# XiSHEN0220/RANSAC-Flow

Hardware: AMD Instinct MI355X
Metric: aligned image-pairs/sec @480×640, 1/2/4/8 MI355X; max-abs flow Δ vs ref (higher is better)
Workload: dtype f32

## Files before the change

include/rfx_api.h:

```cpp
#ifndef RFX_API_H
#define RFX_API_H

#include <stddef.h>
#include <stdint.h>

#ifdef __cplusplus
extern "C" {
#endif

#define RFX_OK 0
#define RFX_E_ARG (-1)
#define RFX_E_LIMIT (-2)

#define RFX_ACT_NONE 0
#define RFX_ACT_RELU 1
#define RFX_ACT_SIGMOID 2

const char* rfx_version(void);

#define RFX_ABI_VERSION 14
int rfx_abi_version(void);

int rfx_group_begin(void);
int rfx_group_end(void* stream);
int rfx_group_abort(void);
int rfx_group_side_streams(int enable);

int rfx_conv2d_f32(const float* in, const float* wT, const int32_t* ktab, const float* scale,
                   const float* shift, const float* residual, float* out, int N, int Cin, int Hin,
                   int Win, int Cout, int KH, int KW, int stride, int pad, int act, void* stream);

int rfx_conv2d_tile_variant(int N, int Cout, int Hout, int Wout);

int rfx_conv2d_kernel_id(int N, int Cin, int Cout, int KH, int KW, int stride, int pad, int Hout, int Wout);

int rfx_conv3x3_f32(const float* in, const float* wP, const float* scale, const float* shift, const float* residual,
                    float* out, int N, int Cin, int H, int W, int Cout, int act, int k_chunk, void* stream);
int rfx_conv3x3_kernel_id(int N, int Cin, int Cout, int H, int W, int k_chunk);
int rfx_conv3x3_s2_f32(const float* in, const float* wP, const float* scale, const float* shift, const float* residual,
                       float* out, int N, int Cin, int H, int W, int Cout, int act, void* stream);

int rfx_conv3x3_conv1x1_kernel_id(int N, int H, int W, int Cmid);
int rfx_conv3x3_conv1x1_f32(const float* in, const float* wP2, const float* scale2, const float* shift2, int act2,
                            const float* wQ3, const float* scale3, const float* shift3, const float* residual, int act3,
                            float* out, int N, int Cin, int H, int W, int Cmid, int Cexp, void* stream);

int rfx_maxpool2d_f32(const float* in, float* out, int NC, int Hin, int Win, int k, int stride,
                      int pad, void* stream);

int rfx_blurpool2d_f32(const float* in, float* out, int NC, int Hin, int Win, int stride, void* stream);

int rfx_maxblurpool2d_f32(const float* in, float* out, int NC, int Hin, int Win, int stride, void* stream);

int rfx_stem_conv3x3_maxblur_f32(const float* in, const float* wT, const float* scale, const float* shift, float* out,
                                 int N, int H, int W, int Cout, void* stream);

int rfx_stem_conv7x7_maxpool_f32(const float* in, const float* wT, const float* scale, const float* shift, float* out,
                                 int N, int H, int W, int Cout, void* stream);

int rfx_l2norm_nchw_f32(const float* in, float* out, int N, int C, int HW, long long out_batch_stride,
                        long long out_chan_stride, void* stream);
int rfx_l2norm_nchw_scatter_f32(const float* in, float* out, int N, int C, int HW, const long long* dst_off,
                                long long out_chan_stride, void* stream);

int rfx_flow_head_f32(const float* logits, float* flow, int N, int K, int rows, int cols, void* stream);

int rfx_resize_bilinear_f32(const float* in, float* out, int NC, int Hin, int Win, int Hout, int Wout,
                            int align_corners, void* stream);

int rfx_lanczos_pass_u8(const uint8_t* in, uint8_t* out, int N, int inH, int inW, int outH, int outW, int C,
                        const int32_t* bounds, const int32_t* weights, int ksize, int vertical, int row_offset,
                        void* stream);

int rfx_u8_to_f32_chw(const uint8_t* in, float* raw, float* norm, int N, int H, int W, const float* mean3_host,
                      const float* std3_host, void* stream);

int rfx_copy_cols_f32(const float* src, float* dst, long long rows, int w_src, int w_dst, void* stream);

int rfx_corr_neigh_f32(const float* x, const float* y, float* out, int N, int C, int H, int W, int K,
                       void* stream);
int rfx_corr_neigh_variant_f32(const float* x, const float* y, float* out, int N, int C, int H, int W, int K,
                               int variant, void* stream);

int rfx_corr_neigh_bidir_f32(const float* x, const float* y, float* out_xy, float* out_yx, int N, int C, int H, int W, int K,
                             void* stream);
int rfx_corr_timing(int enable);
int rfx_corr_timing_collect(float* us_out, int cap);

int rfx_warp_grid_f32(const float* Hm, float* grid, int B, int h, int w, void* stream);

int rfx_grid_sample_f32(const float* in, const float* grid, float* out, int N, int C, int Hi, int Wi,
                        int Ho, int Wo, int align_corners, void* stream);

int rfx_compose_flow_f32(const float* flowDown, const float* coarseGrid, float* flow12, float* inb,
                         float* flowUp, int N, int hd, int wd, int Hc, int Wc, int H, int W, int clamp, void* stream);

int rfx_flow_grad_clamp_f32(const float* flowCoarse, const float* grid, float* flowGrad, float* flow, int B, int H, int W,
                            int grid_batch, void* stream);

int rfx_merge_multi_h_f32(const float* flow, const float* match12, long long match12_stride, const float* cyc,
                          const float* inb, int n, long long HW, float th, int multiH, float* flowGlobal,
                          float* matchGlobal, uint8_t* binary, void* stream);

int rfx_match_score_f32(const float* match12, long long match12_stride, const float* cyc, const float* inb, int n,
                        long long HW, float* score, void* stream);

size_t rfx_remove_small_cc_ws_bytes(int N, int H, int W);
int rfx_remove_small_cc_f32(const float* in, float* out, int N, int H, int W, float match_th, int max_area, void* ws,
                            void* stream);

size_t rfx_remove_small_cc_ragged_ws_bytes(long long total_px);
int rfx_remove_small_cc_ragged_f32(const float* in, float* out, const long long* match_off, const int32_t* dims, int n_active,
                                   long long total_px, long long max_hw, float match_th, void* ws, void* stream);

size_t rfx_mutual_nn_ws_bytes(int nA, int nB);
int rfx_mutual_nn_f32(const float* featA, int ldA, int nA, const float* featB, int ldB, int nB, int C,
                      const float* maskB, int64_t* idx1, int64_t* idx2, int32_t* count, void* ws, int score_chunk,
                      void* stream);

int rfx_mutual_nn_batched_f32(const float* featA, int ldA, int nA, long long strideA, const float* featB, int ldB,
                              int nB, long long strideB, int C, const float* maskB, int64_t* idx1, int64_t* idx2,
                              int32_t* count, void* ws, int batch, int score_chunk, void* stream);

int rfx_mutual_nn_ragged_f32(const float* featA, int ldA, const float* featB, int ldB, const int32_t* nA, const int32_t* nB,
                             int maxNA, int maxNB, int C, const float* maskB, int64_t* idx1, int64_t* idx2, int cap,
                             int32_t* count, void* ws, int batch, int score_chunk, void* stream);

int rfx_dlt4_homography(const float* X, const float* Y, int N, float* Hout, void* stream);

int rfx_prediction_f32(const float* match1, const float* match2, int n, const float* Hs, int N, float* err,
                       void* stream);

int rfx_score_hypotheses(const float* match1, const float* match2, int n, const int64_t* samples, int N,
                         float tol, float* Hout, int64_t* counts, uint8_t* flags_out, void* ws, void* stream);

size_t rfx_ransac_ws_bytes(int n, int N);
int rfx_ransac_h4(const float* match1, const float* match2, int n, const int64_t* samples, int N,
                  float tol, float* bestH, uint8_t* inlier, int32_t* result, void* ws, void* stream);

size_t rfx_ransac_batched_ws_bytes(int cap, int N, int batch);
int rfx_ransac_h4_batched(const float* match1, const float* match2, const int32_t* n, int cap, const int64_t* samples,
                          int N, float tol, float* bestH, uint8_t* inlier, int32_t* result, void* ws, int batch,
                          void* stream);

int rfx_ransac_h4_batched_stage(const float* match1, const float* match2, const int32_t* n, int cap, const int64_t* samples,
                                int N, float tol, float* bestH, uint8_t* inlier, int32_t* result, void* ws, int batch,
                                int stages, void* stream);
int rfx_ransac_degenerate_list(const void* ws, int cap, int N, int batch, int32_t* idx, int32_t* count, int kcap, void* stream);
int rfx_ransac_patch_h(void* ws, int cap, int N, int batch, const int32_t* idx, const int32_t* count, const float* Hpatch,
                       int kcap, void* stream);
int rfx_ransac_degenerate_gather(const void* ws, const float* match1, const float* match2, const int32_t* n, int cap,
                                 const int64_t* samples, int N, int batch, int32_t* idx, int32_t* count, int32_t* off,
                                 int32_t* off_host, float* xy_rows, int row_cap, void* stream);
int rfx_ransac_patch_h_rows(void* ws, int cap, int N, int batch, const int32_t* idx, const int32_t* count, const int32_t* off,
                            const float* H_rows, int row_cap, void* stream);
int rfx_dlt4_homography_flags(const float* X, const float* Y, int N, float* Hout, uint8_t* flags, void* stream);

int rfx_gather_matches_f32(const int64_t* idx1, const int64_t* idx2, const int32_t* n, int cap, const float* xa,
                           const float* ya, const float* xb, const float* yb, float* match1, float* match2, int batch,
                           void* stream);

int rfx_gather_matches_ragged_f32(const int64_t* idx1, const int64_t* idx2, const int32_t* n, int cap, const float* xa,
                                  const float* ya, const long long* offA, const float* xb, const float* yb, const long long* offB,
                                  float* match1, float* match2, int batch, void* stream);

int rfx_draw_samples_i64(const int32_t* n, int64_t* samples, int N, int batch, uint64_t seed, uint64_t stream_id,
                         const int32_t* pair_ids, void* stream);

int rfx_keep_mask_f32(const float* mask, const float* bg, const int32_t* active, int n_active, int h, int w, int rt, int ct,
                      float* keep, void* stream);

int rfx_filter_matches_f32(const int64_t* idx1, const int64_t* idx2, const int32_t* count, int cap, const int32_t* active,
                           int n_active, const float* mask, const float* bg, int h, int w, int rt, int ct, const float* xa,
                           const float* ya, const float* xb, const float* yb, float* match1, float* match2, int32_t* n_out,
                           int32_t* kept, void* stream);

size_t rfx_multih_accept_ws_bytes(int n_active);
int rfx_multih_accept_f32(const float* match, float* mask, const float* bg, const int32_t* active, int n_active, int h, int w,
                          const int32_t* ransac_result, const int32_t* n_match, int32_t* nbH, double th, int mode,
                          int32_t* accept, float* gain, void* ws, const float* bestH, const float* flowDown8,
                          const float* match12Down8, const float* match21Down8, int h8, int w8, const float* flowD2, int hd2,
                          int wd2, float* rec, long long rec_stride, int max_h, int off_H, int off_flow, int off_match,
                          int off_d2, void* stream);

int rfx_filter_matches_ragged_f32(const int64_t* idx1, const int64_t* idx2, const int32_t* count, int cap, const int32_t* active,
                                  int n_active, const float* mask, const float* bg, const long long* moff, const int32_t* geom,
                                  const float* xa, const float* ya, const long long* offA, const float* xb, const float* yb,
                                  const long long* offB, float* match1, float* match2, int32_t* n_out, int32_t* kept,
                                  void* stream);

size_t rfx_multih_accept_ragged_ws_bytes(int n_active);
int rfx_multih_accept_ragged_f32(const float* match, const long long* match_off, float* mask, const float* bg,
                                 const long long* moff, const int32_t* geom, const int32_t* active, int n_active, long long max_hw,
                                 const int32_t* ransac_result, const int32_t* n_match, int32_t* nbH, double th, int mode,
                                 int32_t* accept, float* gain, void* ws, const float* bestH, const float* flowDown8,
                                 const float* match12Down8, const float* match21Down8, const long long* off8, float* rec,
                                 long long rec_stride, int max_h, int off_H, int off_flow, void* stream);

int rfx_multih_accept_ragged_d2_f32(const float* match, const long long* match_off, float* mask, const float* bg,
                                    const long long* moff, const int32_t* geom, const int32_t* active, int n_active,
                                    long long max_hw, const int32_t* ransac_result, const int32_t* n_match, int32_t* nbH, double th,
                                    int mode, int32_t* accept, float* gain, void* ws, const float* bestH, const float* flowDown8,
                                    const float* match12Down8, const float* match21Down8, const long long* off8,
                                    const float* flowD2, const long long* offd2, const int32_t* d2dims, float* rec,
                                    long long rec_stride, int max_h, int off_H, int off_flow, void* stream);

int rfx_conv1x1_split_f32(const float* in, const void* wS, const float* scale, const float* shift, const float* residual,
                          float* out, int N, int Cin, int HW, int Cout, int act, void* stream);
int rfx_conv1x1_split_strided_f32(const float* in, const void* wS, const float* scale, const float* shift, const float* residual,
                                  float* out, int N, int Cin, int Hin, int Win, int Cout, int stride, int act, void* stream);
int rfx_conv1x1_split_tile_channels(int N, int Cin, int HWout, int Cout);
int rfx_conv3x3_split_f32(const float* in, const void* wS3, const float* scale, const float* shift, const float* residual,
                          float* out, int N, int Cin, int H, int W, int Cout, int act, void* stream);
int rfx_conv3x3_split_s2_f32(const float* in, const void* wS3, const float* scale, const float* shift, const float* residual,
                             float* out, int N, int Cin, int H, int W, int Cout, int act, void* stream);

int rfx_conv2d_dilated_f32(const float* in, const float* wT, const int32_t* ktab, const float* scale,
                           const float* shift, const float* residual, float* out, int N, int Cin, int Hin,
                           int Win, int Cout, int KH, int KW, int stride, int pad, int dilation, int act, void* stream);
int rfx_adaptive_avgpool2d_f32(const float* in, float* out, int NC, int Hin, int Win, int Hout, int Wout, void* stream);
int rfx_softmax_accum_f32(const float* logits, float* scores, int N, int C, long long HW, float div, int accumulate, void* stream);
int rfx_argmax_mask_f32(const float* scores, int N, int C, long long HW, int id, int complement, float* mask, int32_t* pred,
                        void* stream);

#ifdef __cplusplus
}
#endif
#endif
```

ransac-flow_amd/rfx/_lib.py:

```python
import ctypes
import os
from ctypes import c_int, c_int32, c_int64, c_uint64, c_float, c_double, c_void_p, c_size_t, c_longlong, c_char_p

_HERE = os.path.dirname(os.path.abspath(__file__))
LIB_PATH = os.environ.get("RFX_LIB") or os.path.normpath(os.path.join(_HERE, "..", "librfx.so"))

SIGNATURES = {
    "rfx_version": (c_char_p, []),
    "rfx_abi_version": (c_int, []),
    "rfx_group_begin": (c_int, []),
    "rfx_group_end": (c_int, [c_void_p]),
    "rfx_group_abort": (c_int, []),
    "rfx_group_side_streams": (c_int, [c_int]),
    "rfx_conv2d_f32": (c_int, [c_void_p] * 7 + [c_int] * 10 + [c_void_p]),
    "rfx_conv2d_dilated_f32": (c_int, [c_void_p] * 7 + [c_int] * 11 + [c_void_p]),
    "rfx_conv1x1_split_f32": (c_int, [c_void_p] * 6 + [c_int] * 5 + [c_void_p]),
    "rfx_conv3x3_split_f32": (c_int, [c_void_p] * 6 + [c_int] * 6 + [c_void_p]),
    "rfx_conv3x3_split_s2_f32": (c_int, [c_void_p] * 6 + [c_int] * 6 + [c_void_p]),
    "rfx_conv1x1_split_strided_f32": (c_int, [c_void_p] * 6 + [c_int] * 7 + [c_void_p]),
    "rfx_conv1x1_split_tile_channels": (c_int, [c_int] * 4),
    "rfx_adaptive_avgpool2d_f32": (c_int, [c_void_p, c_void_p] + [c_int] * 5 + [c_void_p]),
    "rfx_softmax_accum_f32": (c_int, [c_void_p, c_void_p, c_int, c_int, c_longlong, c_float, c_int, c_void_p]),
    "rfx_argmax_mask_f32": (c_int, [c_void_p, c_int, c_int, c_longlong, c_int, c_int, c_void_p, c_void_p, c_void_p]),
    "rfx_conv2d_tile_variant": (c_int, [c_int] * 4),
    "rfx_conv2d_kernel_id": (c_int, [c_int] * 9),
    "rfx_conv3x3_f32": (c_int, [c_void_p] * 6 + [c_int] * 7 + [c_void_p]),
    "rfx_conv3x3_kernel_id": (c_int, [c_int] * 6),
    "rfx_conv3x3_s2_f32": (c_int, [c_void_p] * 6 + [c_int] * 6 + [c_void_p]),
    "rfx_conv3x3_conv1x1_kernel_id": (c_int, [c_int] * 4),
    "rfx_conv3x3_conv1x1_f32": (c_int, [c_void_p] * 4 + [c_int] + [c_void_p] * 4 + [c_int, c_void_p] + [c_int] * 6 + [c_void_p]),
    "rfx_maxpool2d_f32": (c_int, [c_void_p, c_void_p] + [c_int] * 6 + [c_void_p]),
    "rfx_blurpool2d_f32": (c_int, [c_void_p, c_void_p] + [c_int] * 4 + [c_void_p]),
    "rfx_maxblurpool2d_f32": (c_int, [c_void_p, c_void_p] + [c_int] * 4 + [c_void_p]),
    "rfx_stem_conv3x3_maxblur_f32": (c_int, [c_void_p] * 5 + [c_int] * 4 + [c_void_p]),
    "rfx_stem_conv7x7_maxpool_f32": (c_int, [c_void_p] * 5 + [c_int] * 4 + [c_void_p]),
    "rfx_l2norm_nchw_f32": (c_int, [c_void_p, c_void_p, c_int, c_int, c_int, c_longlong, c_longlong, c_void_p]),
    "rfx_l2norm_nchw_scatter_f32": (c_int, [c_void_p, c_void_p, c_int, c_int, c_int, c_void_p, c_longlong, c_void_p]),
    "rfx_flow_head_f32": (c_int, [c_void_p, c_void_p] + [c_int] * 4 + [c_void_p]),
    "rfx_resize_bilinear_f32": (c_int, [c_void_p, c_void_p] + [c_int] * 6 + [c_void_p]),
    "rfx_lanczos_pass_u8": (c_int, [c_void_p, c_void_p] + [c_int] * 6 + [c_void_p, c_void_p] + [c_int] * 3 + [c_void_p]),
    "rfx_u8_to_f32_chw": (c_int, [c_void_p] * 3 + [c_int] * 3 + [c_void_p] * 3),
    "rfx_copy_cols_f32": (c_int, [c_void_p, c_void_p, c_longlong, c_int, c_int, c_void_p]),
    "rfx_corr_neigh_f32": (c_int, [c_void_p] * 3 + [c_int] * 5 + [c_void_p]),
    "rfx_corr_neigh_variant_f32": (c_int, [c_void_p] * 3 + [c_int] * 6 + [c_void_p]),
    "rfx_corr_neigh_bidir_f32": (c_int, [c_void_p] * 4 + [c_int] * 5 + [c_void_p]),
    "rfx_corr_timing": (c_int, [c_int]),
    "rfx_corr_timing_collect": (c_int, [c_void_p, c_int]),
    "rfx_warp_grid_f32": (c_int, [c_void_p, c_void_p] + [c_int] * 3 + [c_void_p]),
    "rfx_grid_sample_f32": (c_int, [c_void_p] * 3 + [c_int] * 7 + [c_void_p]),
    "rfx_compose_flow_f32": (c_int, [c_void_p] * 5 + [c_int] * 8 + [c_void_p]),
    "rfx_flow_grad_clamp_f32": (c_int, [c_void_p] * 4 + [c_int] * 4 + [c_void_p]),
    "rfx_merge_multi_h_f32": (c_int, [c_void_p, c_void_p, c_longlong, c_void_p, c_void_p, c_int, c_longlong, c_float, c_int,
                                      c_void_p, c_void_p, c_void_p, c_void_p]),
    "rfx_match_score_f32": (c_int, [c_void_p, c_longlong, c_void_p, c_void_p, c_int, c_longlong, c_void_p, c_void_p]),
    "rfx_remove_small_cc_ws_bytes": (c_size_t, [c_int] * 3),
    "rfx_remove_small_cc_f32": (c_int, [c_void_p, c_void_p, c_int, c_int, c_int, c_float, c_int, c_void_p, c_void_p]),
    "rfx_remove_small_cc_ragged_ws_bytes": (c_size_t, [c_longlong]),
    "rfx_remove_small_cc_ragged_f32": (c_int, [c_void_p] * 4 + [c_int, c_longlong, c_longlong, c_float, c_void_p, c_void_p]),
    "rfx_mutual_nn_ws_bytes": (c_size_t, [c_int, c_int]),
    "rfx_mutual_nn_f32": (c_int, [c_void_p, c_int, c_int, c_void_p, c_int, c_int, c_int] + [c_void_p] * 5 + [c_int, c_void_p]),
    "rfx_mutual_nn_batched_f32": (c_int, [c_void_p, c_int, c_int, c_longlong, c_void_p, c_int, c_int, c_longlong, c_int]
                                  + [c_void_p] * 5 + [c_int, c_int, c_void_p]),
    "rfx_mutual_nn_ragged_f32": (c_int, [c_void_p, c_int, c_void_p, c_int, c_void_p, c_void_p, c_int, c_int, c_int, c_void_p,
                                         c_void_p, c_void_p, c_int, c_void_p, c_void_p, c_int, c_int, c_void_p]),
    "rfx_dlt4_homography": (c_int, [c_void_p, c_void_p, c_int, c_void_p, c_void_p]),
    "rfx_prediction_f32": (c_int, [c_void_p, c_void_p, c_int, c_void_p, c_int, c_void_p, c_void_p]),
    "rfx_score_hypotheses": (c_int, [c_void_p, c_void_p, c_int, c_void_p, c_int, c_float] + [c_void_p] * 5),
    "rfx_ransac_ws_bytes": (c_size_t, [c_int, c_int]),
    "rfx_ransac_h4": (c_int, [c_void_p, c_void_p, c_int, c_void_p, c_int, c_float] + [c_void_p] * 5),
    "rfx_ransac_batched_ws_bytes": (c_size_t, [c_int, c_int, c_int]),
    "rfx_ransac_h4_batched_stage": (c_int, [c_void_p, c_void_p, c_void_p, c_int, c_void_p, c_int, c_float] + [c_void_p] * 4
                                    + [c_int, c_int, c_void_p]),
    "rfx_ransac_degenerate_list": (c_int, [c_void_p, c_int, c_int, c_int, c_void_p, c_void_p, c_int, c_void_p]),
    "rfx_ransac_patch_h": (c_int, [c_void_p, c_int, c_int, c_int, c_void_p, c_void_p, c_void_p, c_int, c_void_p]),
    "rfx_ransac_degenerate_gather": (c_int, [c_void_p] * 4 + [c_int, c_void_p, c_int, c_int] + [c_void_p] * 5 + [c_int, c_void_p]),
    "rfx_ransac_patch_h_rows": (c_int, [c_void_p, c_int, c_int, c_int] + [c_void_p] * 4 + [c_int, c_void_p]),
    "rfx_dlt4_homography_flags": (c_int, [c_void_p, c_void_p, c_int, c_void_p, c_void_p, c_void_p]),
    "rfx_ransac_h4_batched": (c_int, [c_void_p, c_void_p, c_void_p, c_int, c_void_p, c_int, c_float] + [c_void_p] * 4
                              + [c_int, c_void_p]),
    "rfx_gather_matches_f32": (c_int, [c_void_p, c_void_p, c_void_p, c_int] + [c_void_p] * 6 + [c_int, c_void_p]),
    "rfx_gather_matches_ragged_f32": (c_int, [c_void_p, c_void_p, c_void_p, c_int] + [c_void_p] * 8 + [c_int, c_void_p]),
    "rfx_draw_samples_i64": (c_int, [c_void_p, c_void_p, c_int, c_int, c_uint64, c_uint64, c_void_p, c_void_p]),
    "rfx_filter_matches_f32": (c_int, [c_void_p, c_void_p, c_void_p, c_int, c_void_p, c_int, c_void_p, c_void_p] + [c_int] * 4
                               + [c_void_p] * 9),
    "rfx_keep_mask_f32": (c_int, [c_void_p] * 3 + [c_int] * 5 + [c_void_p, c_void_p]),
    "rfx_multih_accept_ws_bytes": (c_size_t, [c_int]),
    "rfx_multih_accept_f32": (c_int, [c_void_p] * 4 + [c_int] * 3 + [c_void_p] * 3 + [c_double, c_int] + [c_void_p] * 7
                              + [c_int, c_int, c_void_p, c_int, c_int, c_void_p, c_longlong] + [c_int] * 5 + [c_void_p]),
    "rfx_filter_matches_ragged_f32": (c_int, [c_void_p, c_void_p, c_void_p, c_int, c_void_p, c_int] + [c_void_p] * 15),
    "rfx_multih_accept_ragged_ws_bytes": (c_size_t, [c_int]),
    "rfx_multih_accept_ragged_f32": (c_int, [c_void_p] * 7 + [c_int, c_longlong] + [c_void_p] * 3 + [c_double, c_int]
                                     + [c_void_p] * 9 + [c_longlong] + [c_int] * 3 + [c_void_p]),
    "rfx_multih_accept_ragged_d2_f32": (c_int, [c_void_p] * 7 + [c_int, c_longlong] + [c_void_p] * 3 + [c_double, c_int]
                                        + [c_void_p] * 12 + [c_longlong] + [c_int] * 3 + [c_void_p]),
}

ABI_VERSION = 14

_lib = None


def load():
    global _lib
    if _lib is not None:
        return _lib
    import torch
    if not os.path.exists(LIB_PATH):
        raise RuntimeError(
            "librfx.so not found at %s -- build it with `python -c 'import __graft_entry__ as g; g.build()'` "
            "(hipcc --offload-arch=gfx950).  There is no CPU fallback." % LIB_PATH)
    lib = ctypes.CDLL(LIB_PATH)
    for name, (res, args) in SIGNATURES.items():
        try:
            fn = getattr(lib, name)
        except AttributeError as e:
            raise RuntimeError("librfx.so is missing symbol %s (stale build?)" % name) from e
        fn.restype = res
        fn.argtypes = args
    if lib.rfx_abi_version() != ABI_VERSION:
        raise RuntimeError("librfx.so has ABI revision %d, this binding was written against %d (stale build?): rebuild with "
                           "`make -C ransac-flow_amd/csrc`" % (lib.rfx_abi_version(), ABI_VERSION))
    _lib = lib
    return lib


class RfxError(RuntimeError):
    pass


def check(rc, what):
    if rc != 0:
        kind = "bad argument" if rc == -1 else ("limit exceeded" if rc == -2 else "hipError_t %d" % rc)
        raise RfxError("%s failed: %s" % (what, kind))
```

ransac-flow_amd/rfx/nets.py:

```python
import os

import torch

from . import ops
from .ops import ConvPlan, ACT_NONE, ACT_RELU, ACT_SIGMOID


def _bn(sd, p):
    return {k: sd[p + "." + k] for k in ("weight", "bias", "running_mean", "running_var")}


class ResNet50Trunk:

    def __init__(self, sd, device="cuda"):
        self.conv1 = ConvPlan(sd["conv1.weight"], _bn(sd, "bn1"), stride=2, pad=3, act=ACT_RELU, device=device)
        self.blocks = []
        for layer, nblk, stride in (("layer1", 3, 1), ("layer2", 4, 2), ("layer3", 6, 2)):
            for b in range(nblk):
                p = "%s.%d" % (layer, b)
                s = stride if b == 0 else 1
                w1, w2, w3 = (sd["%s.conv%d.weight" % (p, i)] for i in (1, 2, 3))
                tail = ops.bottleneck_tail_shape(ops.ConvGeometry(*w2.shape, stride=s, pad=1, act=ACT_RELU, scale="bn2"),
                                                 ops.ConvGeometry(*w3.shape, stride=1, pad=0, act=ACT_RELU, scale="bn3"))
                if not tail:
                    split2 = split3 = True
                elif ops.conv_split_enabled() and os.environ.get("RFX_SPLIT_TAILS", "1") != "0":
                    split2, split3 = True, w3.shape[1] >= 128
                else:
                    split2 = split3 = False
                blk = {
                    "c1": ConvPlan(w1, _bn(sd, p + ".bn1"), 1, 0, ACT_RELU, device, split=w1.shape[1] >= 128),
                    "c2": ConvPlan(w2, _bn(sd, p + ".bn2"), s, 1, ACT_RELU, device, split=split2),
                    "c3": ConvPlan(w3, _bn(sd, p + ".bn3"), 1, 0, ACT_RELU, device, split=split3),
                    "ds": None,
                }
                if (p + ".downsample.0.weight") in sd:
                    wd = sd[p + ".downsample.0.weight"]
                    blk["ds"] = ConvPlan(wd, _bn(sd, p + ".downsample.1"), s, 0, ACT_NONE, device, split=wd.shape[1] >= 128)
                if tail:
                    blk["c2"].k_chunk = 4
                self.blocks.append(blk)

    def __call__(self, x):
        x = ops.stem_conv7_maxpool(x, self.conv1)
        for blk in self.blocks:
            o = blk["c1"](x)
            r = blk["ds"](x) if blk["ds"] is not None else x
            if ops.bottleneck_tail_eligible(blk["c2"], blk["c3"]):
                x = ops.bottleneck_tail(o, blk["c2"], blk["c3"], residual=r)
            else:
                o = blk["c2"](o)
                x = blk["c3"](o, residual=r)
        return x


    def forward_group(self, xs, side_streams=True):
        dev = xs[0].device
        with ops.launch_group(dev, side_streams):
            xs = [ops.stem_conv7_maxpool(x, self.conv1) for x in xs]
        for blk in self.blocks:
            with ops.launch_group(dev, side_streams):
                os_ = [blk["c1"](x) for x in xs]
                rs = [blk["ds"](x) for x in xs] if blk["ds"] is not None else xs
            if ops.bottleneck_tail_eligible(blk["c2"], blk["c3"]):
                with ops.launch_group(dev, side_streams):
                    ys = [ops.bottleneck_tail(o, blk["c2"], blk["c3"], residual=r) for o, r in zip(os_, rs)]
            else:
                with ops.launch_group(dev, side_streams):
                    ms = [blk["c2"](o) for o in os_]
                with ops.launch_group(dev, side_streams):
                    ys = [blk["c3"](m, residual=r) for m, r in zip(ms, rs)]
            xs = ys
        return xs


class FeatureExtractorNet:

    def __init__(self, sd, device="cuda"):
        self.conv1 = ConvPlan(sd["conv1.weight"], _bn(sd, "bn1"), 1, 1, ACT_RELU, device)
        self.blocks = []
        for layer, stride in (("layer1", 1), ("layer2", 2), ("layer3", 2)):
            for b in range(2):
                p = "%s.%d" % (layer, b)
                s = stride if b == 0 else 1
                blk = {
                    "c1": ConvPlan(sd[p + ".conv1.weight"], _bn(sd, p + ".bn1"), s, 1, ACT_RELU, device, split=True),
                    "c2": ConvPlan(sd[p + ".conv2.weight"], _bn(sd, p + ".bn2"), 1, 1, ACT_RELU, device, split=True),
                    "ds": None, "stride": s,
                }
                if (p + ".downsample.1.weight") in sd:
                    blk["ds"] = ConvPlan(sd[p + ".downsample.1.weight"], _bn(sd, p + ".downsample.2"), 1, 0, ACT_NONE,
                                         device)
                self.blocks.append(blk)

    def __call__(self, x):
        x = ops.stem_conv_maxblur(x, self.conv1)
        for blk in self.blocks:
            o = blk["c1"](x)
            r = blk["ds"](ops.blurpool2d(x, blk["stride"])) if blk["ds"] is not None else x
            x = blk["c2"](o, residual=r)
        return x


class _HeadTrunk:
    def __init__(self, sd, last_act, device):
        self.c1 = ConvPlan(sd["conv1.weight"], _bn(sd, "bn1"), 1, 1, ACT_RELU, device, split=True)
        self.c2 = ConvPlan(sd["conv2.weight"], _bn(sd, "bn2"), 1, 1, ACT_RELU, device, split=True)
        self.c3 = ConvPlan(sd["conv3.weight"], _bn(sd, "bn3"), 1, 1, ACT_RELU, device, split=True)
        self.c4 = ConvPlan(sd["conv4.weight"], None, 1, 1, last_act, device)

    def __call__(self, coef):
        return self.c4(self.c3(self.c2(self.c1(coef))))


class NetFlowCoarseNet:

    def __init__(self, sd, kernelSize=7, device="cuda"):
        self.k = kernelSize
        self.trunk = _HeadTrunk(sd, ACT_NONE, device)

    def __call__(self, coef, up8X=True):
        flow = ops.flow_head(self.trunk(coef), self.k)
        if up8X:
            flow = ops.resize_bilinear(flow, (flow.shape[2] * 8, flow.shape[3] * 8), align_corners=True)
        return flow


class NetMatchabilityNet:

    def __init__(self, sd, kernelSize=7, device="cuda"):
        self.trunk = _HeadTrunk(sd, ACT_SIGMOID, device)

    def __call__(self, feat, up8X=True):
        m = self.trunk(feat)
        if up8X:
            m = ops.resize_bilinear(m, (m.shape[2] * 8, m.shape[3] * 8), align_corners=True)
        return m
```

ransac-flow_amd/rfx/ops.py:

```python
import collections
import ctypes
import os
import threading

import torch

from . import _lib

ACT_NONE, ACT_RELU, ACT_SIGMOID = 0, 1, 2


def _stream(dev=None):
    return ctypes.c_void_p(torch.cuda.current_stream(dev).cuda_stream)


def _on_device(dev, fn, *args):
    if dev.index is not None and dev.index != torch.cuda.current_device():
        with torch.cuda.device(dev):
            return fn(*args, _stream(dev))
    return fn(*args, _stream())


def _call(name, dev, *args):
    _lib.check(_on_device(dev, getattr(_lib.load(), name), *args), name)
# ... 210 lines not shown
        dev = self._device = device or "cuda"
        self.wS = self.wP = self.wT = self.ktab = None
        if self.route == "split1x1":
            self.wS = split_weights(w.reshape(self.Cout, self.Cin)).to(dev)
        elif self.route in ("split3x3", "split3x3_s2"):
            self.wS = split_weights_3x3(w).to(dev)
        else:
            self.wT, self.ktab = pack_wT(w).to(dev), pack_ktab(w, self.dilation).to(dev)
            if self.route == "fp32_3x3":
                self.wP = pack_wP(w).to(dev)
        self.w2d = w.reshape(self.Cout, self.Cin) if (self.KH == 1 and self.KW == 1) else None
        self._wq = None
        if bn is not None:
            invstd = 1.0 / torch.sqrt(bn["running_var"].detach().float().cpu() + eps)
            alpha = bn["weight"].detach().float().cpu() * invstd
            beta = bn["bias"].detach().float().cpu() - bn["running_mean"].detach().float().cpu() * alpha
            self.scale, self.shift = alpha.to(dev), beta.to(dev)
        elif bias is not None:
            self.scale, self.shift = torch.ones(self.Cout, dtype=torch.float32).to(dev), bias.detach().float().cpu().to(dev)
        else:
            self.scale = self.shift = None

    def quad_weights(self):
        if getattr(self, "_wq", None) is None:
            self._wq = pack_wQ(self.w2d).to(self._device)
        return self._wq

    def out_hw(self, H, W):
        eh, ew = (self.KH - 1) * self.dilation + 1, (self.KW - 1) * self.dilation + 1
        return (H + 2 * self.pad - eh) // self.stride + 1, (W + 2 * self.pad - ew) // self.stride + 1

    def __call__(self, x, residual=None, act=None):
        x = _dev(x, "conv input")
        N, C, H, W = x.shape
        if C != self.Cin:
            raise ValueError("conv expects %d input channels, got %d" % (self.Cin, C))
        Ho, Wo = self.out_hw(H, W)
        out = torch.empty((N, self.Cout, Ho, Wo), dtype=torch.float32, device=x.device)
        res = _dev(residual, "residual") if residual is not None else None
        if res is not None and res.shape != out.shape:
            raise ValueError("residual shape %s != output shape %s" % (tuple(res.shape), tuple(out.shape)))
        self._RUN[self.route](self, x, res, out, self.act if act is None else act)
        return out


    def _run_dilated(self, x, res, out, act):
        N, C, H, W = x.shape
        _call("rfx_conv2d_dilated_f32", _one_device(x, res, self.wT), _p(x), _p(self.wT), _p(self.ktab), _p(self.scale), _p(self.shift),
              _p(res), _p(out), N, C, H, W, self.Cout, self.KH, self.KW, self.stride, self.pad, self.dilation, act)

    def _run_split3x3(self, x, res, out, act):
        N, C, H, W = x.shape
        e0 = Profiler.begin(x)
        xin, Cp = x, C
        if C % 16:
            Cp = (C + 15) // 16 * 16
            xin = torch.zeros((N, Cp, H, W), dtype=torch.float32, device=x.device)
            xin[:, :C].copy_(x)
            launch_group.keep(xin)
        _call("rfx_conv3x3_split_f32" if self.stride == 1 else "rfx_conv3x3_split_s2_f32", _one_device(xin, res, self.wS), _p(xin),
              _p(self.wS), _p(self.scale), _p(self.shift), _p(res), _p(out), N, Cp, H, W, self.Cout, act)
        if e0 is not None:
            Ho, Wo = out.shape[2:]
            Profiler.record_conv(KID_SPLIT_3X3 | (2 if self.Cout > 64 else 1) | (4 if self.stride != 1 else 0),
                                 2.0 * N * Ho * Wo * self.Cout * self.Cin * 9, e0, (N, self.Cin, H, W, self.Cout, 3, self.stride),
                                 4.0 * (N * C * H * W + N * self.Cout * Ho * Wo * (2 if res is not None else 1)) + 54.0 * self.Cout * self.Cin)

    def _run_split1x1(self, x, res, out, act):
        N, C, H, W = x.shape
        e0 = Profiler.begin(x)
        if self.stride == 1:
            _call("rfx_conv1x1_split_f32", _one_device(x, res, self.wS), _p(x), _p(self.wS), _p(self.scale), _p(self.shift), _p(res), _p(out),
                  N, C, H * W, self.Cout, act)
        else:
            _call("rfx_conv1x1_split_strided_f32", _one_device(x, res, self.wS), _p(x), _p(self.wS), _p(self.scale), _p(self.shift), _p(res),
                  _p(out), N, C, H, W, self.Cout, self.stride, act)
        if e0 is not None:
            Ho, Wo = out.shape[2:]
            Profiler.record_conv(KID_SPLIT_1X1 | (2 if self.Cout > 64 else 1) | (4 if self.stride != 1 else 0),
                                 2.0 * N * Ho * Wo * self.Cout * self.Cin, e0, (N, self.Cin, H, W, self.Cout, 1, self.stride),
                                 4.0 * (N * C * Ho * Wo + N * self.Cout * Ho * Wo * (2 if res is not None else 1)) + 6.0 * self.Cout * self.Cin)

    def _run_fp32_3x3(self, x, res, out, act):
        N, C, H, W = x.shape
        Ho, Wo = out.shape[2:]
        lib = _lib.load()
        kid0 = (lib.rfx_conv3x3_kernel_id(N, self.Cin, self.Cout, Ho, Wo, self.k_chunk) if self.stride == 1 else
                lib.rfx_conv2d_kernel_id(N, self.Cin, self.Cout, self.KH, self.KW, self.stride, self.pad, Ho, Wo))
        if not kid0 & (KID_DIRECT_3X3 | KID_DIRECT_3X3_S2):
            return self._run_gemm(x, res, out, act)
        e0 = Profiler.begin(x)
        if kid0 & KID_DIRECT_3X3:
            _call("rfx_conv3x3_f32", _one_device(x, res, self.wP), _p(x), _p(self.wP), _p(self.scale), _p(self.shift),
                  _p(res), _p(out), N, C, H, W, self.Cout, act, self.k_chunk)
        else:
            _call("rfx_conv3x3_s2_f32", _one_device(x, res, self.wP), _p(x), _p(self.wP), _p(self.scale), _p(self.shift),
                  _p(res), _p(out), N, C, H, W, self.Cout, act)
        if e0 is not None:
            self._record_fp32(kid0, e0, x, res, out)

    def _run_gemm(self, x, res, out, act):
        N, C, H, W = x.shape
        e0 = Profiler.begin(x)
        _call("rfx_conv2d_f32", _one_device(x, res, self.wT), _p(x), _p(self.wT), _p(self.ktab), _p(self.scale),
              _p(self.shift), _p(res), _p(out), N, C, H, W, self.Cout, self.KH, self.KW, self.stride, self.pad, act)
        if e0 is not None:
            self._record_fp32(0, e0, x, res, out)

    def _record_fp32(self, kid0, e0, x, res, out):
        N, C, H, W = x.shape
        Ho, Wo = out.shape[2:]
        kid = kid0 if (kid0 & KID_DIRECT_3X3) else _lib.load().rfx_conv2d_kernel_id(N, self.Cin, self.Cout, self.KH, self.KW, self.stride, self.pad, Ho, Wo)
        flops = 2.0 * N * Ho * Wo * self.Cout * self.Cin * self.KH * self.KW
        nbytes = 4.0 * (N * C * H * W + N * self.Cout * Ho * Wo * (2 if res is not None else 1)
                        + self.Cout * self.Cin * self.KH * self.KW)
        Profiler.record_conv(kid, flops, e0, (N, self.Cin, H, W, self.Cout, self.KH, self.stride), nbytes)

    _RUN = {"dilated": _run_dilated, "split3x3": _run_split3x3, "split3x3_s2": _run_split3x3, "split1x1": _run_split1x1,
            "fp32_3x3": _run_fp32_3x3, "gemm": _run_gemm}


ConvGeometry = collections.namedtuple("ConvGeometry", "Cout Cin KH KW stride pad act scale")


def bottleneck_tail_shape(plan2, plan3):
    return (plan2.KH == 3 and plan2.KW == 3 and plan2.stride == 1 and plan2.pad == 1 and plan2.Cin % 8 == 0
            and plan2.Cout in (64, 128) and plan2.act in (ACT_NONE, ACT_RELU) and plan3.KH == 1 and plan3.KW == 1
            and plan3.stride == 1 and plan3.pad == 0 and plan3.Cin == plan2.Cout and plan3.Cout % 128 == 0
            and plan3.act in (ACT_NONE, ACT_RELU) and plan3.scale is not None)


def bottleneck_tail_eligible(plan2, plan3):
    return (bottleneck_tail_shape(plan2, plan3) and os.environ.get("RFX_FUSE_BOTTLENECK", "1") != "0"
            and getattr(plan2, "wS", None) is None and getattr(plan3, "wS", None) is None)


def bottleneck_tail(x, plan2, plan3, residual=None):
    x = _dev(x, "bottleneck input")
    N, C, H, W = x.shape
    if C != plan2.Cin:
        raise ValueError("conv expects %d input channels, got %d" % (plan2.Cin, C))
    res = _dev(residual, "residual") if residual is not None else None
    out = torch.empty((N, plan3.Cout, H, W), dtype=torch.float32, device=x.device)
    if res is not None and res.shape != out.shape:
        raise ValueError("residual shape %s != output shape %s" % (tuple(res.shape), tuple(out.shape)))
    e0 = Profiler.begin(x)
    _call("rfx_conv3x3_conv1x1_f32", _one_device(x, res, plan2.wP, plan3.scale), _p(x), _p(plan2.wP), _p(plan2.scale),
          _p(plan2.shift), plan2.act, _p(plan3.quad_weights()), _p(plan3.scale), _p(plan3.shift), _p(res), plan3.act,
          _p(out), N, C, H, W, plan2.Cout, plan3.Cout)
    if e0 is not None:
        Profiler.record_conv(_lib.load().rfx_conv3x3_conv1x1_kernel_id(N, H, W, plan2.Cout),
                             2.0 * N * H * W * (plan2.Cout * plan2.Cin * 9 + plan3.Cout * plan3.Cin), e0, (N, C, H, W, plan3.Cout, 3, 1),
                             4.0 * N * H * W * (C + plan3.Cout * (2 if res is not None else 1)))
    return out


def maxpool2d(x, k, stride, pad=0):
    x = _dev(x, "maxpool input")
    N, C, H, W = x.shape
    Ho, Wo = (H + 2 * pad - k) // stride + 1, (W + 2 * pad - k) // stride + 1
    out = torch.empty((N, C, Ho, Wo), dtype=torch.float32, device=x.device)
    _call("rfx_maxpool2d_f32", x.device, _p(x), _p(out), N * C, H, W, k, stride, pad)
    return out


def blurpool2d(x, stride=2):
    x = _dev(x, "blurpool input")
    N, C, H, W = x.shape
    Ho, Wo = (H - 1) // stride + 1, (W - 1) // stride + 1
    out = torch.empty((N, C, Ho, Wo), dtype=torch.float32, device=x.device)
    _call("rfx_blurpool2d_f32", x.device, _p(x), _p(out), N * C, H, W, stride)
    return out


def maxblurpool2d(x, stride=2):
    x = _dev(x, "maxblurpool input")
    N, C, H, W = x.shape
    Ho, Wo = (H - 2) // stride + 1, (W - 2) // stride + 1
    out = torch.empty((N, C, Ho, Wo), dtype=torch.float32, device=x.device)
    _call("rfx_maxblurpool2d_f32", x.device, _p(x), _p(out), N * C, H, W, stride)
    return out


def stem_conv_maxblur(x, plan):
    x = _dev(x, "stem input")
    N, C, H, W = x.shape
    if not (C == 3 and plan.Cin == 3 and plan.KH == 3 and plan.KW == 3 and plan.stride == 1 and plan.pad == 1
            and plan.act == ACT_RELU and plan.Cout % 32 == 0):
        raise ValueError("stem_conv_maxblur: not a 3x3/s1/p1 ReLU convolution of a 3-channel image")
    Ho, Wo = (H - 2) // 2 + 1, (W - 2) // 2 + 1
    out = torch.empty((N, plan.Cout, Ho, Wo), dtype=torch.float32, device=x.device)
    e0 = Profiler.begin(x)
    _call("rfx_stem_conv3x3_maxblur_f32", _one_device(x, plan.wT), _p(x), _p(plan.wT), _p(plan.scale), _p(plan.shift), _p(out), N, H, W,
                                                       plan.Cout)
    if e0 is not None:
        Profiler.record_conv(256, 2.0 * N * H * W * plan.Cout * 27, e0, (N, 3, H, W, plan.Cout, 3, 1),
                             4.0 * (N * 3 * H * W + N * plan.Cout * Ho * Wo))
    return out


def stem_conv7_maxpool(x, plan):
    x = _dev(x, "stem input")
    N, C, H, W = x.shape
    if not (C == 3 and plan.Cin == 3 and plan.KH == 7 and plan.KW == 7 and plan.stride == 2 and plan.pad == 3
            and plan.act == ACT_RELU and plan.Cout % 32 == 0):
        raise ValueError("stem_conv7_maxpool: not a 7x7/s2/p3 ReLU convolution of a 3-channel image")
    Hc, Wc = (H - 1) // 2 + 1, (W - 1) // 2 + 1
    Hp, Wp = (Hc - 1) // 2 + 1, (Wc - 1) // 2 + 1
    out = torch.empty((N, plan.Cout, Hp, Wp), dtype=torch.float32, device=x.device)
    e0 = Profiler.begin(x)
    _call("rfx_stem_conv7x7_maxpool_f32", _one_device(x, plan.wT), _p(x), _p(plan.wT), _p(plan.scale), _p(plan.shift), _p(out), N, H, W,
                                                       plan.Cout)
    if e0 is not None:
        Profiler.record_conv(257, 2.0 * N * Hc * Wc * plan.Cout * 147, e0, (N, 3, H, W, plan.Cout, 7, 2),
                             4.0 * (N * 3 * H * W + N * plan.Cout * Hp * Wp))
    return out


def adaptive_avgpool2d(x, size):
    x = _dev(x, "adaptive_avgpool input")
    N, C, H, W = x.shape
    Ho, Wo = (int(size), int(size)) if isinstance(size, int) else (int(size[0]), int(size[1]))
    out = torch.empty((N, C, Ho, Wo), dtype=torch.float32, device=x.device)
    _call("rfx_adaptive_avgpool2d_f32", x.device, _p(x), _p(out), N * C, H, W, Ho, Wo)
    return out


def softmax_accum(logits, scores=None, div=1.0):
    logits = _dev(logits, "logits")
    N, C = logits.shape[0], logits.shape[1]
    HW = logits.numel() // (N * C)
    acc = scores is not None
    if acc:
        if not scores.is_contiguous() or scores.shape != logits.shape or scores.dtype != torch.float32 or not scores.is_cuda:
            raise ValueError("scores must be a contiguous float32 device tensor of the logits' shape (updated in place)")
    else:
        scores = torch.empty_like(logits)
    _call("rfx_softmax_accum_f32", _one_device(logits, scores), _p(logits), _p(scores), N, C, HW, float(div), 1 if acc else 0)
    return scores


def argmax_mask(scores, class_id, complement=False, want_pred=False):
    scores = _dev(scores, "scores")
    N, C, H, W = scores.shape
    mask = torch.empty((N, H, W), dtype=torch.float32, device=scores.device)
    pred = torch.empty((N, H, W), dtype=torch.int32, device=scores.device) if want_pred else None
    _call("rfx_argmax_mask_f32", scores.device, _p(scores), N, C, H * W, int(class_id), 1 if complement else 0, _p(mask), _p(pred))
    return (mask, pred) if want_pred else mask


def l2norm(x, out=None, out_batch_stride=0, out_chan_stride=0):
    x = _dev(x, "l2norm input")
    N, C = x.shape[0], x.shape[1]
    HW = x.numel() // (N * C)
    if out is None:
        out = torch.empty_like(x)
        obs = ocs = 0
    else:
        if not out.is_cuda or out.dtype != torch.float32:
            raise TypeError("l2norm out must be a float32 device tensor")
        obs, ocs = out_batch_stride, out_chan_stride
    _call("rfx_l2norm_nchw_f32", _one_device(x, out), _p(x), _p(out), N, C, HW, obs, ocs)
    return out



def l2norm_scatter(x, out, dst_off, out_chan_stride):
    x = _dev(x, "l2norm input")
    if not isinstance(out, torch.Tensor) or not out.is_cuda or out.dtype != torch.float32:
        raise TypeError("l2norm_scatter out must be a float32 device tensor")
    dst_off = _dev(dst_off, "dst_off", torch.int64)
    N, C = x.shape[0], x.shape[1]
    HW = x.numel() // (N * C)
    if dst_off.numel() != N:
        raise ValueError("dst_off must hold one offset per image")
    _call("rfx_l2norm_nchw_scatter_f32", _one_device(x, out, dst_off), _p(x), _p(out), N, C, HW, _p(dst_off), int(out_chan_stride))
    return out

def flow_head(logits, K=7):
    logits = _dev(logits, "flow logits")
    N, C, R, Cc = logits.shape
    if C != K * K:
        raise ValueError("flow head expects %d logits, got %d" % (K * K, C))
    out = torch.empty((N, 2, R, Cc), dtype=torch.float32, device=logits.device)
    _call("rfx_flow_head_f32", logits.device, _p(logits), _p(out), N, K, R, Cc)
    return out


def resize_bilinear(x, size, align_corners=False):
    x = _dev(x, "resize input")
    N, C, H, W = x.shape
    Ho, Wo = int(size[0]), int(size[1])
    out = torch.empty((N, C, Ho, Wo), dtype=torch.float32, device=x.device)
    _call("rfx_resize_bilinear_f32", x.device, _p(x), _p(out), N * C, H, W, Ho, Wo, 1 if align_corners else 0)
    return out


_LANCZOS_TABLES = collections.OrderedDict()
_LANCZOS_MAX = 64


def lanczos_resize_u8(img, out_w, out_h):
    from . import lanczos
    img = _dev(img, "image", torch.uint8)
    N, H, W, C = img.shape
    p = lanczos.plan(W, H, out_w, out_h)
# ... 794 lines not shown
```

Measured before the change: 161.8.

## Add MFMA conv1x1 64→256 expansion kernel fused with downsample shortcut

Adds a new HIP kernel for 1x1 convolutions with 64 input and 256 output channels. It keeps the full weight matrix in LDS and uses 32x32x2 f32 MFMA. A dual variant computes the downsample shortcut conv and the expansion conv in one pass and sums them, so the shortcut tensor is never written to and re-read from memory. The ResNet block loop routes eligible layer1 blocks to it above a pixel threshold. This adds large LDS use (up to 128KB for the dual form), which limits occupancy, and it falls back to the old path inside launch groups.

```diff
diff --git a/include/rfx_api.h b/include/rfx_api.h
--- a/include/rfx_api.h
+++ b/include/rfx_api.h
@@ -18,7 +18,7 @@
 
 const char* rfx_version(void);
 
-#define RFX_ABI_VERSION 14
+#define RFX_ABI_VERSION 15
 int rfx_abi_version(void);
 
 int rfx_group_begin(void);
@@ -215,6 +215,12 @@
 int rfx_conv3x3_split_s2_f32(const float* in, const void* wS3, const float* scale, const float* shift, const float* residual,
                              float* out, int N, int Cin, int H, int W, int Cout, int act, void* stream);
 
+int rfx_conv1x1_expand64_f32(const float* in, const float* wT, const float* scale, const float* shift, const float* residual,
+                             float* out, int N, int Cin, int HW, int Cout, int stride, int act, void* stream);
+int rfx_conv1x1_expand64_dual_f32(const float* in_a, const float* wT_a, const float* scale_a, const float* shift_a,
+                                  const float* in_b, const float* wT_b, const float* scale_b, const float* shift_b, float* out,
+                                  int N, int Cin, int HW, int Cout, int stride, void* stream);
+
 int rfx_conv2d_dilated_f32(const float* in, const float* wT, const int32_t* ktab, const float* scale,
                            const float* shift, const float* residual, float* out, int N, int Cin, int Hin,
                            int Win, int Cout, int KH, int KW, int stride, int pad, int dilation, int act, void* stream);
diff --git a/ransac-flow_amd/csrc/conv1x1e.hip b/ransac-flow_amd/csrc/conv1x1e.hip
--- /dev/null
+++ b/ransac-flow_amd/csrc/conv1x1e.hip
@@ -0,0 +1,146 @@
+#include "common.h"
+#include "conv_epilogue.h"
+#include "group.h"
+#include <type_traits>
+
+namespace {
+
+constexpr int E64_K = 64;
+constexpr int E64_MAXC = 256;
+constexpr int E64_WAVES = 8;
+constexpr int E64_PIX = 32;
+constexpr int E64_PLAIN_NS = 4, E64_DUAL_NS = 2;
+
+struct E64Args {
+    const float* in[2]; const float* wT[2]; const float* scale[2]; const float* shift[2];
+    const float* res; float* out;
+    int HW, Cout, act;
+    long long P;
+    long long tiles;
+};
+
+template <bool TWO, int NS>
+__global__ __launch_bounds__(E64_WAVES * 64) void conv1x1_expand64_kernel(E64Args a) {
+    constexpr int SRC = TWO ? 2 : 1;
+    __shared__ __attribute__((aligned(16))) float Ws[SRC][E64_K][E64_MAXC];
+    __shared__ float s_scale[SRC][E64_MAXC], s_shift[SRC][E64_MAXC];
+
+    const int t = threadIdx.x, lane = t & 63, wave = t >> 6;
+    const int lrow = lane >> 5, lcol = lane & 31;
+    const size_t HW = (size_t)a.HW;
+
+    const int c4 = a.Cout / 4;
+#pragma unroll
+    for (int s = 0; s < SRC; ++s) {
+        for (int i = t; i < E64_K * c4; i += E64_WAVES * 64) {
+            const int k = i / c4, c = i - k * c4;
+            *reinterpret_cast<f32x4*>(&Ws[s][k][c * 4]) = *reinterpret_cast<const f32x4*>(a.wT[s] + (size_t)k * a.Cout + c * 4);
+        }
+        if (t < a.Cout) {
+            s_scale[s][t] = a.scale[s] ? a.scale[s][t] : 1.0f;
+            s_shift[s][t] = a.shift[s] ? a.shift[s][t] : 0.0f;
+        }
+    }
+    __syncthreads();
+
+    const long long stride = (long long)gridDim.x * E64_WAVES;
+    for (long long tile = (long long)blockIdx.x * E64_WAVES + wave; tile < a.tiles; tile += stride) {
+        long long pp = tile * E64_PIX + lcol;
+        bool pix_ok[1] = {pp < a.P};
+        if (!pix_ok[0]) pp = a.P - 1;
+        const long long n = pp / a.HW;
+        const size_t hw = (size_t)(pp - n * a.HW);
+        const size_t in_off = ((size_t)n * E64_K + lrow) * HW + hw;
+        size_t pix_off[1] = {(size_t)n * a.Cout * HW + hw};
+
+        float xv[SRC][E64_K / 2];
+#pragma unroll
+        for (int s = SRC - 1; s >= 0; --s)
+#pragma unroll
+            for (int kk = 0; kk < E64_K / 2; ++kk) xv[s][kk] = a.in[s][in_off + (size_t)(2 * kk) * HW];
+
+        for (int m0 = 0; m0 < a.Cout; m0 += 32 * NS) {
+            auto gemm = [&](auto src, f32x16 (&acc)[NS][1]) {
+                constexpr int s = decltype(src)::value;
+                const float* wp = &Ws[s][lrow][m0 + lcol];
+#pragma unroll
+                for (int i = 0; i < NS; ++i)
+#pragma unroll
+                    for (int r = 0; r < 16; ++r) acc[i][0][r] = 0.0f;
+#pragma unroll
+                for (int kk = 0; kk < E64_K / 2; ++kk)
+#pragma unroll
+                    for (int i = 0; i < NS; ++i)
+                        acc[i][0] = __builtin_amdgcn_mfma_f32_32x32x2f32(wp[2 * kk * E64_MAXC + i * 32], xv[s][kk], acc[i][0], 0, 0, 0);
+            };
+            float d[NS][16];
+            f32x16 acc[NS][1];
+            if constexpr (TWO) {
+                gemm(std::integral_constant<int, 1>(), acc);
+#pragma unroll
+                for (int i = 0; i < NS; ++i) {
+                    const int ml0 = m0 + i * 32 + 4 * lrow;
+#pragma unroll
+                    for (int r = 0; r < 16; ++r)
+                        d[i][r] = fmaf(acc[i][0][r], s_scale[1][ml0 + (r & 3) + 8 * (r >> 2)], s_shift[1][ml0 + (r & 3) + 8 * (r >> 2)]);
+                }
+            }
+            gemm(std::integral_constant<int, 0>(), acc);
+            conv_epilogue<NS, 1, false, TWO>(acc, s_scale[0] + m0, s_shift[0] + m0, TWO ? a.out : a.res, a.out, a.act, a.Cout, HW, m0, 0,
+                                             lrow, pix_off, pix_ok, true, d);
+        }
+    }
+}
+
+template <bool TWO, int NS>
+int launch_e64(const E64Args& a, hipStream_t st) {
+    static int cus = 0;
+    if (!cus) {
+        int dev = 0;
+        cus = 256;
+        if (hipGetDevice(&dev) == hipSuccess) (void)hipDeviceGetAttribute(&cus, hipDeviceAttributeMultiprocessorCount, dev);
+    }
+    const long long wgs = (a.tiles + E64_WAVES - 1) / E64_WAVES;
+    const unsigned grid = (unsigned)(wgs < cus ? wgs : cus);
+    hipLaunchKernelGGL((conv1x1_expand64_kernel<TWO, NS>), dim3(grid), dim3(E64_WAVES * 64), 0, st, a);
+    RFX_LAUNCH_CHECK();
+    return RFX_OK;
+}
+
+int e64_check(int N, int Cin, int HW, int Cout, int stride, int act) {
+    if (N <= 0 || HW <= 0) return RFX_E_ARG;
+    if (Cin != E64_K || stride != 1 || Cout <= 0 || Cout % E64_MAXC != 0) return RFX_E_ARG;
+    if (Cout > E64_MAXC) return RFX_E_LIMIT;
+    if (act != RFX_ACT_NONE && act != RFX_ACT_RELU) return RFX_E_ARG;
+    if (rfx_group_recording()) return RFX_E_ARG;
+    return RFX_OK;
+}
+
+}
+
+extern "C" int rfx_conv1x1_expand64_f32(const float* in, const float* wT, const float* scale, const float* shift,
+                                        const float* residual, float* out, int N, int Cin, int HW, int Cout, int stride, int act,
+                                        void* stream) {
+    if (!in || !wT || !out) return RFX_E_ARG;
+    if (const int rc = e64_check(N, Cin, HW, Cout, stride, act)) return rc;
+    E64Args a{};
+    a.in[0] = in; a.wT[0] = wT; a.scale[0] = scale; a.shift[0] = shift;
+    a.res = residual; a.out = out; a.HW = HW; a.Cout = Cout; a.act = act;
+    a.P = (long long)N * HW;
+    a.tiles = (a.P + E64_PIX - 1) / E64_PIX;
+    return launch_e64<false, E64_PLAIN_NS>(a, rfx_stream(stream));
+}
+
+extern "C" int rfx_conv1x1_expand64_dual_f32(const float* in_a, const float* wT_a, const float* scale_a, const float* shift_a,
+                                             const float* in_b, const float* wT_b, const float* scale_b, const float* shift_b,
+                                             float* out, int N, int Cin, int HW, int Cout, int stride, void* stream) {
+    if (!in_a || !wT_a || !in_b || !wT_b || !out) return RFX_E_ARG;
+    if (const int rc = e64_check(N, Cin, HW, Cout, stride, RFX_ACT_RELU)) return rc;
+    E64Args a{};
+    a.in[0] = in_a; a.wT[0] = wT_a; a.scale[0] = scale_a; a.shift[0] = shift_a;
+    a.in[1] = in_b; a.wT[1] = wT_b; a.scale[1] = scale_b; a.shift[1] = shift_b;
+    a.res = nullptr; a.out = out; a.HW = HW; a.Cout = Cout; a.act = RFX_ACT_RELU;
+    a.P = (long long)N * HW;
+    a.tiles = (a.P + E64_PIX - 1) / E64_PIX;
+    return launch_e64<true, E64_DUAL_NS>(a, rfx_stream(stream));
+}
diff --git a/ransac-flow_amd/rfx/_lib.py b/ransac-flow_amd/rfx/_lib.py
--- a/ransac-flow_amd/rfx/_lib.py
+++ b/ransac-flow_amd/rfx/_lib.py
@@ -19,6 +19,8 @@
     "rfx_conv3x3_split_s2_f32": (c_int, [c_void_p] * 6 + [c_int] * 6 + [c_void_p]),
     "rfx_conv1x1_split_strided_f32": (c_int, [c_void_p] * 6 + [c_int] * 7 + [c_void_p]),
     "rfx_conv1x1_split_tile_channels": (c_int, [c_int] * 4),
+    "rfx_conv1x1_expand64_f32": (c_int, [c_void_p] * 6 + [c_int] * 6 + [c_void_p]),
+    "rfx_conv1x1_expand64_dual_f32": (c_int, [c_void_p] * 9 + [c_int] * 5 + [c_void_p]),
     "rfx_adaptive_avgpool2d_f32": (c_int, [c_void_p, c_void_p] + [c_int] * 5 + [c_void_p]),
     "rfx_softmax_accum_f32": (c_int, [c_void_p, c_void_p, c_int, c_int, c_longlong, c_float, c_int, c_void_p]),
     "rfx_argmax_mask_f32": (c_int, [c_void_p, c_int, c_int, c_longlong, c_int, c_int, c_void_p, c_void_p, c_void_p]),
@@ -95,7 +97,7 @@
                                         + [c_void_p] * 12 + [c_longlong] + [c_int] * 3 + [c_void_p]),
 }
 
-ABI_VERSION = 14
+ABI_VERSION = 15
 
 _lib = None
 
diff --git a/ransac-flow_amd/rfx/nets.py b/ransac-flow_amd/rfx/nets.py
--- a/ransac-flow_amd/rfx/nets.py
+++ b/ransac-flow_amd/rfx/nets.py
@@ -45,13 +45,25 @@
         x = ops.stem_conv7_maxpool(x, self.conv1)
         for blk in self.blocks:
             o = blk["c1"](x)
+            form = self.expand64_form(blk)
+            if form == "dual":
+                x = ops.conv1x1_expand64(blk["c2"](o), blk["c3"], shortcut=(x, blk["ds"]))
+                continue
             r = blk["ds"](x) if blk["ds"] is not None else x
             if ops.bottleneck_tail_eligible(blk["c2"], blk["c3"]):
                 x = ops.bottleneck_tail(o, blk["c2"], blk["c3"], residual=r)
+            elif form == "plain":
+                x = ops.conv1x1_expand64(blk["c2"](o), blk["c3"], residual=r)
             else:
                 o = blk["c2"](o)
                 x = blk["c3"](o, residual=r)
         return x
+
+    @staticmethod
+    def expand64_form(blk):
+        if ops.bottleneck_tail_eligible(blk["c2"], blk["c3"]):
+            return None
+        return ops.expand64_form(blk["c3"], blk["ds"])
 
 
     def forward_group(self, xs, side_streams=True):
diff --git a/ransac-flow_amd/rfx/ops.py b/ransac-flow_amd/rfx/ops.py
--- a/ransac-flow_amd/rfx/ops.py
+++ b/ransac-flow_amd/rfx/ops.py
@@ -386,6 +386,75 @@
         Profiler.record_conv(_lib.load().rfx_conv3x3_conv1x1_kernel_id(N, H, W, plan2.Cout),
                              2.0 * N * H * W * (plan2.Cout * plan2.Cin * 9 + plan3.Cout * plan3.Cin), e0, (N, C, H, W, plan3.Cout, 3, 1),
                              4.0 * N * H * W * (C + plan3.Cout * (2 if res is not None else 1)))
+    return out
+
+
+_EXPAND64 = None
+
+
+def expand64_enabled():
+    global _EXPAND64
+    if _EXPAND64 is None:
+        _EXPAND64 = os.environ.get("RFX_EXPAND64", "1") != "0"
+    return _EXPAND64
+
+
+def expand64_eligible(plan):
+    return (plan.KH == 1 and plan.KW == 1 and plan.stride == 1 and plan.pad == 0 and getattr(plan, "dilation", 1) == 1
+            and plan.Cin == 64 and plan.Cout % 256 == 0 and plan.Cout <= 256 and plan.scale is not None
+            and plan.act in (ACT_NONE, ACT_RELU))
+
+
+EXPAND64_MIN_PIXELS = {"plain": 300000, "dual": 100000}
+
+
+def expand64_form(plan3, plan_ds=None, pixels=None):
+    def ok(p):
+        return expand64_eligible(p) and getattr(p, "route", "gemm") == "gemm"
+    if not expand64_enabled() or not ok(plan3) or plan3.act != ACT_RELU:
+        return None
+    if plan_ds is not None:
+        form = "dual" if (ok(plan_ds) and plan_ds.act == ACT_NONE and plan_ds.Cout == plan3.Cout) else None
+    else:
+        form = "plain"
+    if form is not None and pixels is not None and pixels < EXPAND64_MIN_PIXELS[form]:
+        return None
+    return form
+
+
+def conv1x1_expand64(x, plan, residual=None, shortcut=None):
+    if residual is not None and shortcut is not None:
+        raise ValueError("conv1x1_expand64: a residual or a shortcut, not both")
+    x = _dev(x, "conv input")
+    N, C, H, W = x.shape
+    plan_s = shortcut[1] if shortcut is not None else None
+    form = expand64_form(plan, plan_s, N * H * W)
+    if getattr(launch_group._tls, "active", None) is not None:
+        form = None
+    if form is None:
+        return plan(x, residual=plan_s(shortcut[0]) if shortcut is not None else residual)
+    if C != plan.Cin:
+        raise ValueError("conv expects %d input channels, got %d" % (plan.Cin, C))
+    out = torch.empty((N, plan.Cout, H, W), dtype=torch.float32, device=x.device)
+    e0 = Profiler.begin(x)
+    if form == "dual":
+        xs = _dev(shortcut[0], "shortcut input")
+        if xs.shape != x.shape:
+            raise ValueError("shortcut input shape %s != conv input shape %s" % (tuple(xs.shape), tuple(x.shape)))
+        _call("rfx_conv1x1_expand64_dual_f32", _one_device(x, xs, plan.wT, plan_s.wT), _p(x), _p(plan.wT), _p(plan.scale), _p(plan.shift),
+              _p(xs), _p(plan_s.wT), _p(plan_s.scale), _p(plan_s.shift), _p(out), N, C, H * W, plan.Cout, 1)
+    else:
+        res = _dev(residual, "residual") if residual is not None else None
+        if res is not None and res.shape != out.shape:
+            raise ValueError("residual shape %s != output shape %s" % (tuple(res.shape), tuple(out.shape)))
+        _call("rfx_conv1x1_expand64_f32", _one_device(x, res, plan.wT), _p(x), _p(plan.wT), _p(plan.scale), _p(plan.shift), _p(res), _p(out),
+              N, C, H * W, plan.Cout, 1, plan.act)
+    if e0 is not None:
+        gemms = 2 if form == "dual" else 1
+        planes = plan.Cout * (2 if (form == "plain" and residual is not None) else 1)
+        Profiler.record_conv(_lib.load().rfx_conv2d_kernel_id(N, plan.Cin, plan.Cout, 1, 1, 1, 0, H, W),
+                             gemms * 2.0 * N * H * W * plan.Cout * plan.Cin, e0, (N, plan.Cin, H, W, plan.Cout, 1, 1),
+                             4.0 * (N * H * W * (gemms * C + planes) + gemms * plan.Cout * plan.Cin))
     return out
 
 
```

After: 164.8 (median of 6 runs). 1.02x the previous value.
